# Starlight0798/gymRL

Measured on AMD Instinct MI355X. Metric: env-steps/sec at N envs/GPU (PPO LunarLander), 1/2/4/8 GPUs + %HBM roofline, higher is better.
Workload: dtype f32; 1 GPU; PPO LunarLander-v3, 4096 vectorised envs per MI355X (BASELINE.json configs[1]); envs_per_gpu=4096, rollout_len=2048, num_epochs=10, num_minibatches=32, minibatch=262144, model=ActorCritic 8-256-256-{256-4,256-1} tanh, 200,965 params, parallelism=single GPU

## Files before the change

### gymrl_amd/_lib.py

```python
import ctypes as C
import os
import subprocess

import torch

_HERE = os.path.dirname(os.path.abspath(__file__))
LIB_PATH = os.environ.get("GYMRL_HIP_LIB") or os.path.join(_HERE, "libgymrl_hip.so")
CSRC = os.path.join(_HERE, "csrc")

ABI_VERSION = 4

_lib = None

def build(force=False):
    if force:
        subprocess.check_call(["make", "-C", CSRC, "-s", "clean"])
    subprocess.check_call(["make", "-C", CSRC, "-s", "-j8"])
    return LIB_PATH


class LinItem(C.Structure):
    _c_name_ = "gymrl_lin_item"
    _fields_ = ([(n, C.c_void_p) for n in ("x", "x2", "w", "b", "y", "dy", "dx", "dx2", "dw", "db")] +
                [("act", C.c_int), ("lo", C.c_float), ("hi", C.c_float), ("argmax", C.c_void_p)])
# ... 533 lines not shown
    "gymrl_mhc_gates": (_i, [_vp, _vp, _vp, _vp, _vp, _i, _i, _i, _i, _vp, _vp, _vp, _vp, _vp, _vp]),
    "gymrl_mhc_combine": (_i, [_vp, _vp, _vp, _vp, _i, _i, _i, _i, _vp, _vp]),
    "gymrl_rmsnorm": (_i, [_vp, _vp, _i, _i, _i, _f, _i, _vp, _vp]),
    "gymrl_rmsnorm_bwd_workspace_bytes": (_sz, [_i]),
    "gymrl_rmsnorm_bwd": (_i, [_vp, _vp, _vp, _i, _i, _f, _i, _vp, _vp, _vp, _vp]),
    "gymrl_rmsnorm_sum_bwd": (_i, [_vp, _vp, _vp, _i, _i, _i, _f, _i, _vp, _vp, _vp, _vp]),
    "gymrl_norm_proj_fwd": (_i, [_vp, _vp, _vp, _vp, _i, _i, _i, _f, _vp, _vp]),
    "gymrl_norm_proj_bwd_workspace_bytes": (_sz, [_i, _i]),
    "gymrl_norm_proj_bwd": (_i, [_vp, _vp, _vp, _vp, _i, _i, _i, _f, _vp, _vp, _vp, _vp, _vp, _vp]),
    "gymrl_sinkhorn": (_i, [_vp, _i, _i, _i, _vp, _vp, _vp]),
    "gymrl_mhc_gates_bwd_workspace_bytes": (_sz, [_i, _i]),
    "gymrl_mhc_gates_bwd": (_i, [_vp, _vp, _vp, _vp, _vp, _vp, _vp, _vp, _vp, _vp, _vp, _vp, _vp, _i, _i, _i, _vp, _vp, _vp, _vp, _vp, _vp, _vp]),
    "gymrl_mhc_read_fwd": (_i, [_vp, _vp, _i, _i, _i, _vp, _vp]),
    "gymrl_mhc_read_bwd": (_i, [_vp, _vp, _vp, _i, _i, _i, _vp, _vp, _i, _vp]),
    "gymrl_mhc_combine_bwd": (_i, [_vp, _vp, _vp, _vp, _vp, _i, _i, _i, _i, _vp, _vp, _vp, _vp, _vp]),
    "gymrl_mhc_sub_forward": (_i, [_vp, _i, _vp, _vp, _vp, _vp, _vp, _vp, _i, _i, _i, _i, _vp, _vp, _vp, _vp, _vp, _vp, _vp, _vp]),
    "gymrl_mhc_sub_backward": (_i, [_vp, _i, _vp, _i, _vp, _vp, _vp, _vp, _vp, _vp, _vp, _vp, _vp, _i, _i, _i, _vp, _vp, _i, _vp, _vp, _vp, _vp, _vp,
                                    _vp]),
    "gymrl_mhc_policy_image_floats": (_sz, [_i]),
    "gymrl_mhc_policy_pack": (_i, [_vp, _vp, _vp]),
    "gymrl_mhc_policy_forward": (_i, [_vp, _vp, _i, _vp, _vp, _vp]),
    "gymrl_mlp_train_workspace_bytes": (_sz, [_i, _i, _i]),
    "gymrl_linear_tanh_smallk": (_i, [_vp, _vp, _vp, _i64, _i, _i, _vp, _vp]),
    "gymrl_linear_smallk": (_i, [_vp, _vp, _vp, _i64, _i, _i, _vp, _vp]),
    "gymrl_tanh_inplace": (_i, [_vp, _i64, _vp, _i, _vp]),
    "gymrl_tanh_bwd_colsum": (_i, [_vp, _vp, _i64, _i, _vp, _vp, _vp]),
    "gymrl_linear_smallk_bwd": (_i, [_vp, _vp, _vp, _i64, _i, _i, _vp, _vp, _vp, _vp, _vp, _vp]),
    "gymrl_heads_fwd_tanh": (_i, [_vp, _i64, _i, _i, _vp, _vp, _vp, _vp, _vp, _vp, _vp, _i, _vp]),
    "gymrl_heads_bwd": (_i, [_vp, _vp, _vp, _i64, _i, _i, _vp, _vp, _vp, _vp, _vp, _vp, _vp, _vp, _i, _vp, _vp, _vp]),
    "gymrl_heads_loss_blocks": (_i, [_i64, _i]),
    "gymrl_ppo_update_shape_ok": (_i, [_i, _i, _i]),
    "gymrl_heads_loss_fwd_bwd": (_i, [_vp, _i64, _i, _i, _vp, _vp, _vp, _vp, _vp, _vp, _vp, _vp, _vp, _vp, _P(PPOCfg), _vp, _vp, _vp, _vp, _vp, _vp,
                                      _vp, _vp]),
    "gymrl_ppo_gauss_update_shape_ok": (_i, [_i, _i, _i]),
    "gymrl_gauss_heads_loss_workspace_bytes": (_sz, [_i64, _i, _i]),
    "gymrl_gauss_heads_loss_fwd_bwd": (_i, [_vp, _i64, _i, _i, _vp, _vp, _vp, _vp, _vp, _vp, _vp, _vp, _vp, _vp, _vp, _P(PPOCfg), _vp, _vp, _vp,
                                            _vp, _vp, _vp, _vp, _vp, _vp, _i, _vp]),
    "gymrl_gemm_workspace_bytes": (_sz, []),
    "gymrl_linear_fwd": (_i, [_vp, _vp, _vp, _i64, _i, _i, _i, _vp, _vp]),
    "gymrl_linear_bwd_input": (_i, [_vp, _vp, _vp, _i64, _i, _i, _vp, _vp]),
    "gymrl_linear_bwd_input_add": (_i, [_vp, _vp, _vp, _i64, _i, _i, _vp, _vp]),
    "gymrl_linear_geometry": (_i, [_i, _i64, _i, _i, _P(_i), _P(_i)]),
    "gymrl_linear_bwd_weight_geometry": (_i, [_i64, _i, _P(_i), _P(_i64)]),
    "gymrl_linear_bwd_weight": (_i, [_vp, _vp, _i64, _i, _i, _vp, _vp, _vp, _vp]),
    "gymrl_update_finalize": (_i, [_i64, _i, _i, _i, _vp, _vp, _vp, _vp, _vp, _vp, _vp, _vp, _vp, _vp, _vp, _vp, _vp, _vp, _vp]),
    "gymrl_replay_append": (_i, [_vp, _vp, _vp, _vp, _vp, _i64, _i64, _i, _i, _i, _vp, _vp, _vp, _vp, _vp, _vp, _vp]),
# ... 130 lines not shown
```

### gymrl_amd/csrc/finalize_device.hpp

```cpp
#pragma once
#include "train_device.hpp"

namespace gymrl {
namespace fin {

constexpr int kCUs = 256;
constexpr size_t kColsumBytes = (size_t)kCUs * 512 * sizeof(float);

__host__ __device__ __forceinline__ void tn_geometry(int64_t B, int N, int* slices, int64_t* rps) {
  const int ntiles = N / 256;
  int s = kCUs / ntiles;
  int64_t r = (B + s - 1) / s;
  r += r & 1;
  if (r < 64) r = 64;
  s = (int)((B + r - 1) / r);
  if (s < 1) s = 1;
  *slices = s;
  *rps = r;
}

__device__ __forceinline__ void tn_colsum_body(const float* __restrict__ parts, int slices, float* __restrict__ db, int block,
                                               double (*sm)[64]) {
  const int n = block * 64 + (threadIdx.x & 63), j = threadIdx.x >> 6;
  const int ntile = n >> 8, nl = n & 255;
// ... 4 lines not shown
    float v[8];
#pragma unroll
    for (int k = 0; k < 8; ++k) v[k] = src[(size_t)(s + 4 * k) * 256];
#pragma unroll
    for (int k = 0; k < 8; ++k) g += (double)v[k];
  }
  for (; s < slices; s += 4) g += (double)src[(size_t)s * 256];
  sm[j][threadIdx.x & 63] = g;
  __syncthreads();
  if (j == 0) {
    const int l = threadIdx.x;
    db[n] = (float)(((sm[0][l] + sm[1][l]) + sm[2][l]) + sm[3][l]);
  }
}

__device__ __forceinline__ void tn_reduce_body(const float* __restrict__ parts, int slices, int ldw, float* __restrict__ dW,
                                               int block, double (*sm)[64][4]) {
  typedef float f32x4 __attribute__((ext_vector_type(4)));
  const int g = threadIdx.x >> 6, e = block * 64 + (threadIdx.x & 63);
  const int ntile = e >> 14, e4 = e & 16383;
  const f32x4* src = reinterpret_cast<const f32x4*>(parts) + (size_t)ntile * slices * 16384 + e4;
  double s0 = 0.0, s1 = 0.0, s2 = 0.0, s3 = 0.0;
  int s = g;
  for (; s + 12 < slices; s += 16) {
    const f32x4 v0 = src[(size_t)s * 16384], v1 = src[(size_t)(s + 4) * 16384];
    const f32x4 v2 = src[(size_t)(s + 8) * 16384], v3 = src[(size_t)(s + 12) * 16384];
    s0 += (double)v0[0]; s1 += (double)v0[1]; s2 += (double)v0[2]; s3 += (double)v0[3];
    s0 += (double)v1[0]; s1 += (double)v1[1]; s2 += (double)v1[2]; s3 += (double)v1[3];
    s0 += (double)v2[0]; s1 += (double)v2[1]; s2 += (double)v2[2]; s3 += (double)v2[3];
    s0 += (double)v3[0]; s1 += (double)v3[1]; s2 += (double)v3[2]; s3 += (double)v3[3];
  }
  for (; s < slices; s += 4) {
    const f32x4 v = src[(size_t)s * 16384];
    s0 += (double)v[0]; s1 += (double)v[1]; s2 += (double)v[2]; s3 += (double)v[3];
  }
  const int le = threadIdx.x & 63;
  if (g > 0) { sm[g - 1][le][0] = s0; sm[g - 1][le][1] = s1; sm[g - 1][le][2] = s2; sm[g - 1][le][3] = s3; }
  __syncthreads();
  if (g == 0) {
#pragma unroll
    for (int j = 0; j < 3; ++j) { s0 += sm[j][le][0]; s1 += sm[j][le][1]; s2 += sm[j][le][2]; s3 += sm[j][le][3]; }
    const int n = e4 >> 6, k4 = e4 & 63;
    *reinterpret_cast<f32x4*>(dW + (size_t)(ntile * 256 + n) * ldw + 4 * k4) = f32x4{(float)s0, (float)s1, (float)s2, (float)s3};
  }
}

}
}
```

### gymrl_amd/csrc/mlp_train.hip

```cpp
#include "train_device.hpp"
#include "finalize_device.hpp"
#include "policy_device.hpp"
#include "gauss_policy_device.hpp"
#include "../../include/gymrl.h"

namespace {

using namespace gymrl;

constexpr int kTB = 256;
constexpr int kMaxBlocks = 1024;

struct RowMap {
  int lpr, rpw, r_in, c4;
  __device__ RowMap(int C, int lane) : lpr(C >> 2), rpw(64 / (C >> 2)), r_in(lane / (C >> 2)), c4(lane % (C >> 2)) {}
};

inline int grid_for(int64_t rows, int C) {
  const int rows_per_block = (kTB / 64) * (64 / (C / 4));
  int64_t nb = (rows + rows_per_block - 1) / rows_per_block;
  return (int)(nb < kMaxBlocks ? (nb < 1 ? 1 : nb) : kMaxBlocks);
}

template <int NV>
__device__ __forceinline__ void block_colsum(const float (&acc)[NV], int C, const RowMap& m, float* sm,
                                             float* __restrict__ partials) {
  static_assert(NV % 4 == 0, "vectors of 4 columns");
  const int wave = threadIdx.x >> 6;
  const int groups = (kTB / 64) * m.rpw;
  const int g = wave * m.rpw + m.r_in;
  const int width = (NV / 4) * C;
#pragma unroll
  for (int v = 0; v < NV / 4; ++v)
#pragma unroll
    for (int j = 0; j < 4; ++j) sm[(size_t)g * width + v * C + 4 * m.c4 + j] = acc[4 * v + j];
  __syncthreads();
  for (int e = threadIdx.x; e < width; e += kTB) {
    float s = 0.0f;
    for (int gg = 0; gg < groups; ++gg) s += sm[(size_t)gg * width + e];
    partials[(size_t)blockIdx.x * width + e] = s;
  }
}

constexpr int kFinE = 32, kFinB = kTB / kFinE;
__device__ __forceinline__ double reduce_partials(const float* __restrict__ partials, int nblocks, int width, int e,
                                                  bool valid) {
  __shared__ double fin[kFinB][kFinE];
  const int te = threadIdx.x % kFinE, tb = threadIdx.x / kFinE;
  double s = 0.0;
  if (valid) {
    int b = tb;
    for (; b + 3 * kFinB < nblocks; b += 4 * kFinB) {
      const float p0 = partials[(size_t)b * width + e], p1 = partials[(size_t)(b + kFinB) * width + e];
      const float p2 = partials[(size_t)(b + 2 * kFinB) * width + e], p3 = partials[(size_t)(b + 3 * kFinB) * width + e];
      s += (double)p0; s += (double)p1; s += (double)p2; s += (double)p3;
    }
    for (; b < nblocks; b += kFinB) s += (double)partials[(size_t)b * width + e];
  }
  fin[tb][te] = s;
  __syncthreads();
  double t = 0.0;
  if (tb == 0) {
#pragma unroll
    for (int k = 0; k < kFinB; ++k) t += fin[k][te];
  }
  return t;
}

template <int D>
__device__ __forceinline__ void load_row(float (&xv)[D], const float* __restrict__ p) {
  if constexpr (D % 4 == 0) {
#pragma unroll
    for (int d = 0; d < D; d += 4) {
      const f32x4 v = *reinterpret_cast<const f32x4*>(p + d);
      xv[d] = v[0]; xv[d + 1] = v[1]; xv[d + 2] = v[2]; xv[d + 3] = v[3];
    }
  } else if constexpr (D == 6) {
#pragma unroll
// ... 12 lines not shown
                                                                 const float* __restrict__ b, int64_t B, int C,
                                                                 float* __restrict__ out) {
  const RowMap m(C, threadIdx.x & 63);
  float w[4][D], bias[4];
#pragma unroll
  for (int j = 0; j < 4; ++j) {
    bias[j] = b ? b[4 * m.c4 + j] : 0.0f;
#pragma unroll
    for (int d = 0; d < D; ++d) w[j][d] = W[(size_t)(4 * m.c4 + j) * D + d];
  }
  const int64_t stride = (int64_t)gridDim.x * (kTB / 64) * m.rpw;
  for (int64_t r = ((int64_t)blockIdx.x * (kTB / 64) + (threadIdx.x >> 6)) * m.rpw + m.r_in; r < B; r += stride) {
    float xv[D];
    load_row<D>(xv, x + r * D);
    f32x4 o;
#pragma unroll
    for (int j = 0; j < 4; ++j) {
      float acc = 0.0f;
#pragma unroll
      for (int d = 0; d < D; ++d) acc = fmaf(xv[d], w[j][d], acc);
      o[j] = TANH ? train_tanhf(acc + bias[j]) : acc + bias[j];
    }
    __builtin_nontemporal_store(o, reinterpret_cast<f32x4*>(out + r * C + 4 * m.c4));
  }
}

__global__ __launch_bounds__(kTB) void tanh_inplace_kernel(float* __restrict__ z, int64_t n4, const float* __restrict__ bias,
                                                           int C4) {
  f32x4* p = reinterpret_cast<f32x4*>(z);
  for (int64_t i = (int64_t)blockIdx.x * kTB + threadIdx.x; i < n4; i += (int64_t)gridDim.x * kTB) {
    f32x4 v = p[i];
    if (bias) {
      const f32x4 b = reinterpret_cast<const f32x4*>(bias)[i & (C4 - 1)];
#pragma unroll
      for (int j = 0; j < 4; ++j) v[j] += b[j];
    }
#pragma unroll
    for (int j = 0; j < 4; ++j) v[j] = train_tanhf(v[j]);
    p[i] = v;
  }
}

template <int A>
__global__ __launch_bounds__(kTB) void heads_fwd_tanh_kernel(float* __restrict__ Zac, int64_t B, int C,
                                                             const float* __restrict__ bac,
                                                             const float* __restrict__ Wa2, const float* __restrict__ ba2,
// ... 719 lines not shown

extern "C" {

size_t gymrl_mlp_train_workspace_bytes(int C, int D, int A) {
  if (C <= 0 || D < 0 || A < 0) return 0;
  const size_t w1 = (size_t)(D + 1) * C, w2 = (size_t)(3 + A + (A + 1 + 3) / 4) * C;
  return sizeof(float) * kMaxBlocks * (w1 > w2 ? w1 : w2) + 256;
}

int gymrl_linear_tanh_smallk(const float* x, const float* W, const float* b, int64_t B, int D, int C, float* out,
                             void* stream) {
  if (!x || !W || !out || B < 0 || !pow2_cols(C) || !al16(out) || !al16(x)) return -22;
  if (B == 0) return 0;
  const dim3 grid(grid_for(B, C) * 1), block(kTB);
  hipStream_t s = (hipStream_t)stream;
  switch (D) {
    case 2: hipLaunchKernelGGL(linear_tanh_smallk_kernel<2>, grid, block, 0, s, x, W, b, B, C, out); break;
    case 3: hipLaunchKernelGGL(linear_tanh_smallk_kernel<3>, grid, block, 0, s, x, W, b, B, C, out); break;
    case 4: hipLaunchKernelGGL(linear_tanh_smallk_kernel<4>, grid, block, 0, s, x, W, b, B, C, out); break;
    case 6: hipLaunchKernelGGL(linear_tanh_smallk_kernel<6>, grid, block, 0, s, x, W, b, B, C, out); break;
    case 8: hipLaunchKernelGGL(linear_tanh_smallk_kernel<8>, grid, block, 0, s, x, W, b, B, C, out); break;
    default: return -22;
  }
  GYMRL_CHECK_LAUNCH();
  return 0;
}

int gymrl_linear_smallk(const float* x, const float* W, const float* b, int64_t B, int D, int C, float* out, void* stream) {
  if (!x || !W || !out || B < 0 || !pow2_cols(C) || !al16(out) || !al16(x)) return -22;
  if (B == 0) return 0;
  const dim3 grid(grid_for(B, C) * 1), block(kTB);
  hipStream_t s = (hipStream_t)stream;
  switch (D) {
    case 2: hipLaunchKernelGGL((linear_tanh_smallk_kernel<2, false>), grid, block, 0, s, x, W, b, B, C, out); break;
    case 3: hipLaunchKernelGGL((linear_tanh_smallk_kernel<3, false>), grid, block, 0, s, x, W, b, B, C, out); break;
    case 4: hipLaunchKernelGGL((linear_tanh_smallk_kernel<4, false>), grid, block, 0, s, x, W, b, B, C, out); break;
    case 6: hipLaunchKernelGGL((linear_tanh_smallk_kernel<6, false>), grid, block, 0, s, x, W, b, B, C, out); break;
    case 8: hipLaunchKernelGGL((linear_tanh_smallk_kernel<8, false>), grid, block, 0, s, x, W, b, B, C, out); break;
    default: return -22;
  }
  GYMRL_CHECK_LAUNCH();
  return 0;
}

int gymrl_tanh_inplace(float* z, int64_t n, const float* bias, int C, void* stream) {
  if (!z || n < 0 || (n & 3) || !al16(z)) return -22;
// ... 182 lines not shown
```

### gymrl_amd/csrc/ppo.hip

```cpp
#include "gymrl_device.hpp"
#include "policy_device.hpp"
#include "gauss_policy_device.hpp"
#include "../../include/gymrl.h"

using namespace gymrl;

namespace {

constexpr int kBlock = 256;

template <int K, int BLOCK>
__device__ __forceinline__ void block_partials(double (&v)[K], double* __restrict__ partials) {
  __shared__ double sm[K][BLOCK / 64];
  const int lane = threadIdx.x & 63, wid = threadIdx.x >> 6;
#pragma unroll
  for (int k = 0; k < K; ++k) {
    const double s = wave_sum(v[k]);
    if (lane == 0) sm[k][wid] = s;
  }
  __syncthreads();
  if (threadIdx.x < K) {
    double s = 0.0;
#pragma unroll
    for (int w = 0; w < BLOCK / 64; ++w) s += sm[threadIdx.x][w];
    partials[(size_t)blockIdx.x * K + threadIdx.x] = s;
// ... 357 lines not shown
#pragma unroll
  for (int k = 0; k < K; ++k) v[k] = 0.0;
  for (int i = threadIdx.x; i < nblocks; i += kBlock) {
#pragma unroll
    for (int k = 0; k < K; ++k) v[k] += partials[(size_t)i * K + k];
  }
  const int lane = threadIdx.x & 63, wid = threadIdx.x >> 6;
#pragma unroll
  for (int k = 0; k < K; ++k) {
    const double s = wave_sum(v[k]);
    if (lane == 0) sm[k][wid] = s;
  }
  __syncthreads();
  if (threadIdx.x < K) {
    double s = 0.0;
#pragma unroll
    for (int w = 0; w < kBlock / 64; ++w) s += sm[threadIdx.x][w];
    metrics_sum[threadIdx.x] += s;
  }
}

constexpr int kMaxLossBlocks = 1024;

constexpr int kRecF = 16;

__global__ __launch_bounds__(kBlock) void permutation_kernel(uint64_t seed, uint64_t counter, uint32_t M, int a, int b,
                                                             int32_t* __restrict__ out) {
  const uint32_t i = blockIdx.x * kBlock + threadIdx.x;
  if (i < M) out[i] = (int32_t)keyed_permute(i, M, a, b, seed, counter);
}

__global__ __launch_bounds__(kBlock) void pack_rollout_kernel(
    const float* __restrict__ obs, const int32_t* __restrict__ act, const float* __restrict__ logp,
    const float* __restrict__ adv, const float* __restrict__ ret, int64_t M, int D,
    float* __restrict__ packed) {
  const int64_t stride = (int64_t)gridDim.x * kBlock;
  for (int64_t i = (int64_t)blockIdx.x * kBlock + threadIdx.x; i < M; i += stride) {
    float r[kRecF];
#pragma unroll
    for (int k = 0; k < 12; ++k) r[k] = k < D ? obs[i * D + k] : 0.0f;
    r[12] = __int_as_float(act[i]); r[13] = logp[i]; r[14] = adv[i]; r[15] = ret[i];
    float4* dst = reinterpret_cast<float4*>(packed + i * kRecF);
#pragma unroll
    for (int q = 0; q < 4; ++q) dst[q] = make_float4(r[4 * q], r[4 * q + 1], r[4 * q + 2], r[4 * q + 3]);
  }
}

__global__ __launch_bounds__(kBlock) void gather_minibatch_kernel(
    const float* __restrict__ packed, const int32_t* __restrict__ idx, int B, int D,
    float* __restrict__ obs_out, int32_t* __restrict__ act_out, float* __restrict__ logp_out,
    float* __restrict__ adv_out, float* __restrict__ ret_out) {
  for (int b = blockIdx.x * kBlock + threadIdx.x; b < B; b += gridDim.x * kBlock) {
    const float4* src = reinterpret_cast<const float4*>(packed + (size_t)idx[b] * kRecF);
    const float4 q0 = src[0], q1 = src[1], q2 = src[2], q3 = src[3];
    const float r[12] = {q0.x, q0.y, q0.z, q0.w, q1.x, q1.y, q1.z, q1.w, q2.x, q2.y, q2.z, q2.w};
    if (D == 8) {
      reinterpret_cast<float4*>(obs_out)[2 * (size_t)b] = q0;
      reinterpret_cast<float4*>(obs_out)[2 * (size_t)b + 1] = q1;
    } else if (D == 4) {
      reinterpret_cast<float4*>(obs_out)[b] = q0;
    } else {
#pragma unroll
      for (int k = 0; k < 12; ++k) if (k < D) obs_out[(size_t)b * D + k] = r[k];
    }
    act_out[b] = __float_as_int(q3.x); logp_out[b] = q3.y; adv_out[b] = q3.z; ret_out[b] = q3.w;
  }
}

__global__ __launch_bounds__(kBlock) void gather_rows_kernel(const float4* __restrict__ src, const int32_t* __restrict__ idx, int64_t n,
                                                             int quads, float4* __restrict__ out) {
  for (int64_t e = (int64_t)blockIdx.x * kBlock + threadIdx.x; e < n * quads; e += (int64_t)gridDim.x * kBlock) {
    const int64_t b = e / quads;
    const int q = (int)(e - b * quads);
    out[e] = src[(int64_t)idx[b] * quads + q];
  }
}

inline int cdiv(int a, int b) { return (a + b - 1) / b; }

}

#define DISPATCH_A(A_, CALL)              \
  switch (A_) {                           \
    case 2: { constexpr int A = 2; CALL; } break; \
    case 3: { constexpr int A = 3; CALL; } break; \
    case 4: { constexpr int A = 4; CALL; } break; \
    case 5: { constexpr int A = 5; CALL; } break; \
    case 6: { constexpr int A = 6; CALL; } break; \
    case 7: { constexpr int A = 7; CALL; } break; \
// ... 282 lines not shown
```

### gymrl_amd/ops.py

```python
import collections
import ctypes as C

import torch

from ._lib import (ACT_NONE, ACT_RELU, ACT_TANH, MLP_MAX_INPUT, MLP_MAX_STAGES, MLP_MAX_WIDTH, ClassicDuelEvalArgs, ClassicEvalArgs, ClassicPpoEvalArgs, DdqnUpdateArgs, EsNoiseArgs, EsPerturbArgs, EsShapeGradArgs, SnesPerturbArgs, SnesTellArgs, DqnActArgs, NdqnActArgs, NdqnCombineArgs, NdqnUpdateArgs, DqnUpdateArgs, DsacActArgs, DsacUpdateArgs, GaeOnline,
                   LunarCollectArgs, LunarEvalArgs, PendulumPpoEvalArgs, RolloutPendulumArgs, MlpDesc, MlpPackStackArgs, MlprnnParams, AcrobotNetEvalArgs, MountainCarEvalArgs, MountainCarNetEvalArgs, PPOCfg, PPOFullCfg, RainbowActArgs, RainbowUpdateArgs, RolloutLunarArgs, SacActArgs, SacUpdateArgs,
                   TabularTrainArgs, Td3ActArgs, Td3UpdateArgs, check, lib)

_vp = C.c_void_p


def _ptr(t, dtype=None, allow_none=False):
    if t is None:
        if allow_none:
            return _vp(None)
        raise ValueError("tensor required")
    if not t.is_cuda:
        raise RuntimeError("gymrl_amd ops run on the MI355X only: got a CPU tensor (there is no CPU fallback)")
    if dtype is not None and t.dtype != dtype:
        raise TypeError(f"expected {dtype}, got {t.dtype}")
    if not t.is_contiguous():
        raise ValueError("tensor must be contiguous")
    return _vp(t.data_ptr())

# ... 1502 lines not shown
        e.act, e.src, e.dst = int(st.get("act", ACT_NONE)), int(st["src"]), int(st["dst"])
        if e.dst < 0:
            if out is None or out.dim() != 2 or out.shape[1] != e.out_dim:
                raise ValueError("dst == -1 needs an `out` tensor [n_rows, out_dim]")
            e.out, e.out_stride = _ptr(out, torch.float32).value, out.stride(0)
    d._keepalive = list(stages)
    return d


def mlp_forward(x, desc):
    n, in_dim = x.shape
    check(lib().gymrl_mlp_forward(_ptr(x, torch.float32), n, in_dim, C.byref(desc), _stream()), "gymrl_mlp_forward")


def mlp_train_workspace(C_, D, A, device):
    n = lib().gymrl_mlp_train_workspace_bytes(C_, D, A)
    return torch.empty(n, dtype=torch.uint8, device=device)


def linear_tanh_smallk(x, W, b, out):
    B, D = x.shape
    check(lib().gymrl_linear_tanh_smallk(_ptr(x, torch.float32), _ptr(W, torch.float32), _ptr(b, torch.float32, True), B, D, W.shape[0],
                                         _ptr(out, torch.float32), _stream()), "gymrl_linear_tanh_smallk")
    return out


def linear_smallk(x, W, b, out):
    B, D = x.shape
    check(lib().gymrl_linear_smallk(_ptr(x, torch.float32), _ptr(W, torch.float32), _ptr(b, torch.float32, True), B, D, W.shape[0],
                                    _ptr(out, torch.float32), _stream()), "gymrl_linear_smallk")
    return out


def tanh_inplace(z, bias=None):
    check(lib().gymrl_tanh_inplace(_ptr(z, torch.float32), z.numel(), _ptr(bias, torch.float32, True), z.shape[-1], _stream()), "gymrl_tanh_inplace")
    return z


def tanh_bwd_colsum(dH, H, colsum_out, workspace):
    B, Cc = dH.shape
    check(lib().gymrl_tanh_bwd_colsum(_ptr(dH, torch.float32), _ptr(H, torch.float32), B, Cc, _ptr(colsum_out, torch.float32), _ptr(workspace),
                                      _stream()), "gymrl_tanh_bwd_colsum")
    return dH


def linear_smallk_bwd(dH, H, x, dW, db, workspace, W=None, b=None):
# ... 1275 lines not shown
```

### gymrl_amd/ppo_lunarlander.py

```python
from collections import deque

import numpy as np
import torch
import torch.nn as nn

from . import dist as gdist
from . import ops
from .envs import VecEnv
from .flat import FusedAdam, flatten_module
from . import ppo_net
from .nn import FusedMLP, Linear


class Config:
    def __init__(self):
        self.env_name = "LunarLander-v3"
        self.seed = None

        self.max_train_steps = 1_000_000
        self.update_freq = 2048
        self.num_epochs = 10
        self.batch_size = 64
        self.num_minibatches = None

# ... 182 lines not shown
        T = int(config.update_freq)
        self.buffer = self._build_buffer(T, N, state_dim)
        self.step_count = 0
        self.rollout_count = 0
        self.episode_rewards = deque(maxlen=100)
        self._gae_ws = ops.gae_workspace(T, N, self.device)
        self._moments = torch.zeros(3, dtype=torch.float64, device=self.device)
        self._next_value = torch.zeros(N, device=self.device)
        self._perm_seed, self._perm_draws, self._perm = self.base_seed * 7919 + 13 + self.rank, 0, None
        self._loss_cfg = (config.clip_eps, config.dual_clip, config.value_coef, config.entropy_coef)
        self._finished = None
        self._metric_parts = None
        self._agg_ready = self._carry_ready = False
        self._parity_noise = None
        self._parity_indices = []
        self._wg_ticks = None
        self._eval_env_factory = None
        self._gae_running = torch.zeros(2, N, dtype=torch.float64, device=self.device)
        self._packed = None
        mb = self._minibatch_size_for(T * N)
        self._stage = (torch.empty(mb, state_dim, device=self.device), torch.empty(mb, dtype=torch.int32, device=self.device),
                       torch.empty(mb, device=self.device), torch.empty(mb, device=self.device),
                       torch.empty(mb, device=self.device))
        self._stage2 = tuple(torch.empty_like(t) for t in self._stage) if self.collective else None
        self._reducer = None
        self._graph = None
        self._timers = None
        if self.rank == 0:
            print(f"Device: {self.device} x{self.world_size} | envs/GPU: {N} | rollout T: {T}")
            print(f"State dim: {state_dim}, Action dim: {action_dim}")
            print(f"Model parameters: {sum(p.numel() for p in self.model.parameters()):,}")

    def _action_dim(self):
        return self.env.action_space.n

    def _build_model(self, state_dim, action_dim):
        return ActorCritic(state_dim, action_dim, self.cfg.hidden_dim)

    def _build_buffer(self, T, N, state_dim):
        return RolloutBuffer(T, N, state_dim, self.device)

    def _sample_step(self, t, head, value, noise, counter0, online):
        b, env = self.buffer, self.env
        ops.categorical_sample(head, value=value.view(-1), noise_exp=None if noise is None else noise[t],
                               seed=env.seed, counter=counter0 + t,
                               env_id0=env.env_id0, act_out=b.actions[t], logp_out=b.log_probs[t],
                               ent_out=None, value_out=b.values[t], online=online)
# ... 175 lines not shown
                self._timers.stop("moments_allreduce", 3)
        total = len(b)
        mb = self._minibatch_size()
        n_mb = (total + mb - 1) // mb
        obs_dim = b.states.shape[-1]
        tm = self._timers
        self._packed = ops.pack_rollout(b.states[:b.T].reshape(total, obs_dim), self._packed_actions(),
                                        b.log_probs.view(-1), b.advantages.view(-1), b.returns.view(-1),
                                        self._packed)
        fu = self._fused_update_for(mb)
        one_pass = fu is not None
        nblk = fu.metric_blocks(mb) if one_pass else ops.loss_blocks(mb)
        if self._metric_parts is None or self._metric_parts.shape[:2] != (cfg.num_epochs * n_mb, nblk):
            self._metric_parts = torch.zeros(cfg.num_epochs * n_mb, nblk, 5, dtype=torch.float64, device=self.device)
        else:
            self._metric_parts.zero_()
        red = None
        if self.collective:
            if self._reducer is None:
                split = (self.model.actor[0].weight.data_ptr() - self.flat_params.data_ptr()) // 4
                self._reducer = gdist.GradReducer(self.flat_grads, [split] if one_pass else None)
            red = self._reducer
            red.timed = tm is not None
        stages = (self._stage, self._stage2) if red is not None else (self._stage, self._stage)

        def minibatches():
            for epoch in range(cfg.num_epochs):
                if indices is not None:
                    perm = torch.as_tensor(indices[epoch], device=self.device).to(torch.int32)
                else:
                    self._perm_draws += 1
                    self._perm = ops.permutation(self._perm_seed, self._perm_draws, total, self.device,
                                                 out=self._perm if self._perm is not None and self._perm.numel() == total else None)
                    perm = self._perm
                for start in range(0, total, mb):
                    yield perm[start:start + mb]

        def gather(mb_idx, k):
            B = mb_idx.numel()
            if tm is not None:
                tm.start("gather_minibatch")
            out = ops.gather_minibatch(self._packed, mb_idx, obs_dim, stages[k & 1] if B == mb else None)
            if tm is not None:
                tm.stop("gather_minibatch", B)
            return out

        graphed = (one_pass and red is None and bool(getattr(cfg, "use_graphs", False)) and total % mb == 0
                   and cfg.num_epochs * n_mb > 3)
        gs = self._graph_state(fu, mb, obs_dim) if graphed else None

        sizes = []
        row = 0
        it = minibatches()
        first = next(it)
        cur = gather(first, 0) if not graphed else first
        while cur is not None:
            if tm is not None:
                tm.tick()
            if graphed:
                mb_idx = cur
                B = mb_idx.numel()
                if tm is not None and tm.live:
                    fu.timers = tm
                    g5 = gather(mb_idx, 0)
                    fu.step(*g5, self._loss_cfg, self._moments, self._metric_parts[row])
                    tm.start("adam_step")
                    self.optimizer.step(grad_scale=1.0)
                    tm.stop("adam_step", self.flat_params.numel())
                else:
                    fu.timers = None
                    gs["idx"].copy_(mb_idx)
                    gs["scalars"].set(gs["off"], self.optimizer.next_bias())
                    gs["scalars"].flush()
                    gs["step"]()
                    self._metric_parts[row].copy_(gs["metric"])
                sizes.append(B)
                row += 1
                cur = next(it, None)
                continue
            mb_obs, mb_act, mb_lp, mb_adv, mb_ret = cur
            B = mb_obs.shape[0]
            if one_pass:
                fu.step(mb_obs, mb_act, mb_lp, mb_adv, mb_ret, self._loss_cfg, self._moments, self._metric_parts[row],
                        reducer=red)
            else:
                self._loss_backward(mb_obs, mb_act, mb_lp, mb_adv, mb_ret, row, tm)
                if red is not None:
                    red.launch(0)
            nxt = next(it, None)
            cur = gather(nxt, row + 1) if nxt is not None else None
            if red is not None:
                red.wait()
            if tm is not None:
                tm.start("adam_step")
            self.optimizer.step(grad_scale=1.0 / self.world_size)
            if tm is not None:
                tm.stop("adam_step", self.flat_params.numel())
            sizes.append(B)
            row += 1
        if tm is not None:
            tm.resume()
        metrics = ops.reduce_rows(self._metric_parts, row, nblk, 5)
        self._drain_episode_returns()
        m = metrics.cpu().numpy() / np.asarray(sizes, np.float64)[:, None]
        m = m.mean(axis=0)
        return {"policy_loss": m[0], "value_loss": m[1], "entropy": m[2], "clip_frac": m[3], "approx_kl": m[4]}

    def _graph_state(self, fu, mb, obs_dim):
        key = (id(fu), mb, self._packed.data_ptr(), self._stage[0].data_ptr())
        gs = self._graph
        if gs is None or gs["key"] != key:
            from .graphs import GraphedStep, StepScalars
            sc = StepScalars(self.device)
            bias, off = sc.slot(16, torch.float32)
            gs = self._graph = dict(key=key, scalars=sc, bias=bias, off=off,
                                    idx=torch.empty(mb, dtype=torch.int32, device=self.device),
                                    metric=torch.zeros(fu.metric_blocks(mb), 5, dtype=torch.float64, device=self.device))

            def body():
                g5 = ops.gather_minibatch(self._packed, gs["idx"], obs_dim, self._stage)
                fu.step(*g5, self._loss_cfg, self._moments, gs["metric"])
                self.optimizer.step(grad_scale=1.0, bias_dev=gs["bias"])
            gs["step"] = GraphedStep(body, warmup=2)
        return gs

    def save_checkpoint(self, path):
        from .utils import checkpoint
        return checkpoint.save_agent(path, {"model": self.model}, {"optimizer": (self.model, self.optimizer)},
                                     step_count=self.step_count, rollout_count=self.rollout_count,
                                     perm_draws=self._perm_draws, episode_rewards=list(self.episode_rewards))

    def load_checkpoint(self, path):
        from .utils import checkpoint
        rest = checkpoint.load_agent(path, {"model": self.model}, {"optimizer": (self.model, self.optimizer)})
        self.step_count = int(rest.get("step_count", 0))
        self.rollout_count = int(rest.get("rollout_count", 0))
        self._perm_draws = int(rest.get("perm_draws", 0))
        self.episode_rewards.clear()
        self.episode_rewards.extend(rest.get("episode_rewards", []))
        gdist.broadcast(self.flat_params)
        return rest

    def train(self):
        if self.rank == 0:
# ... 116 lines not shown
```

### gymrl_amd/ppo_net.py

```python
import torch

from . import ops

LAYOUT = ["shared.0.weight", "shared.0.bias", "shared.2.weight", "shared.2.bias",
          "actor.0.weight", "critic.0.weight", "actor.0.bias", "critic.0.bias",
          "actor.2.weight", "actor.2.bias", "critic.2.weight", "critic.2.bias"]


def supported(model):
    H = model.shared[0].out_features
    D = model.shared[0].in_features
    A = model.actor[2].out_features
    return (ops.ppo_update_shape_ok(H, D, A)
            and model.shared[2].out_features == H and model.actor[0].out_features == H
            and model.critic[0].out_features == H)


def gauss_supported(model):
    H = model.shared[0].out_features
    D = model.shared[0].in_features
    A = model.actor[2].out_features
    return (ops.ppo_gauss_update_shape_ok(H, D, A)
            and model.shared[2].out_features == H and model.actor[0].out_features == H
            and model.critic[0].out_features == H and hasattr(model, "log_std"))
# ... 15 lines not shown
        if wc.data_ptr() != wa.data_ptr() + wa.numel() * 4 or bc.data_ptr() != ba.data_ptr() + ba.numel() * 4:
            raise ValueError("actor.0 / critic.0 are not adjacent: flatten_module(model, device, order=ppo_net.LAYOUT)")
        flat, gflat = model._flat_params, model._flat_grads

        def view(p, n, shape, buf):
            off = (p.data_ptr() - flat.data_ptr()) // 4
            return buf[off:off + n].view(shape)
        self.Wac = view(wa, 2 * H * H, (2 * H, H), flat)
        self.bac = view(ba, 2 * H, (2 * H,), flat)
        self.dWac = view(wa, 2 * H * H, (2 * H, H), gflat)
        self.dbac = view(ba, 2 * H, (2 * H,), gflat)
        self.ws = ops.mlp_train_workspace(H, self.D, self.A, dev)
        R = int(max_rows)
        self.R = R
        self.H1 = torch.empty(R, H, device=dev)
        self.H2 = torch.empty(R, H, device=dev)
        self.Hac = torch.empty(R, 2 * H, device=dev)
        self.dH2 = torch.empty(R, H, device=dev)
        self.dH1 = torch.empty(R, H, device=dev)
        self.timers = None
        self.one_pass_heads, defer = self._schedule()
        self.gemm_ws = ops.gemm_workspace(dev) if H == 256 else None
        self.defer_finalize = defer
        self.gemm_ws2 = ops.gemm_workspace(dev) if defer else None
        self.ws2 = ops.mlp_train_workspace(H, self.D, self.A, dev) if defer else None
        if not self.one_pass_heads:
            self.logits = torch.empty(R, self.A, device=dev)
            self.value = torch.empty(R, 1, device=dev)
            self.dlogits = torch.empty(R, self.A, device=dev)
            self.dvalue = torch.empty(R, device=dev)
        if H != 256:
            self.lin_ws = ops.lin_workspace(R, 2 * H, H, 1, dev) if R > 512 else None

    def _schedule(self):
        return self.H == 256 or self.A == 3, self.H == 256

    def _heads_one_pass(self, t, sfx, B, Zac, heads, act, logp_old, adv, ret, loss_cfg, adv_moments, dbac, hg, metric_parts):
        t("heads_loss_fwd_bwd" + sfx, B, ops.heads_loss_fwd_bwd, Zac, None, *heads, act, logp_old, adv, ret, loss_cfg, adv_moments,
          dbac, *hg, metric_parts, self.ws)

    def _timed(self, name, units, fn, *args, **kw):
        tm = self.timers
        if tm is None:
            return fn(*args, **kw)
        tm.start(name)
        r = fn(*args, **kw)
        tm.stop(name, units)
        return r

    def metric_blocks(self, B):
        return ops.heads_loss_blocks(B, self.H) if self.one_pass_heads else ops.loss_blocks(B)

    @torch.no_grad()
    def step(self, x, act, logp_old, adv, ret, loss_cfg, adv_moments, metric_parts, reducer=None):
        m, B, H = self.m, x.shape[0], self.H
        if B > self.R:
            raise ValueError("minibatch larger than the buffers")
        t = self._timed
        H1, H2, Zac, dZ2, dZ1 = self.H1[:B], self.H2[:B], self.Hac[:B], self.dH2[:B], self.dH1[:B]
        W2, ws = m.shared[2].weight, self.gemm_ws
        sfx = "" if H == 256 else f"_h{H}"
        t("linear_tanh_smallk", B, ops.linear_tanh_smallk, x, m.shared[0].weight, m.shared[0].bias, H1)
        t(f"gemm_fwd_{H}_tanh", B, ops.linear_fwd, H1, W2, m.shared[2].bias, H2, True)
        t(f"gemm_fwd_{2 * H}", B, ops.linear_fwd, H2, self.Wac, self.bac, Zac, False)
        heads = (m.actor[2].weight, m.actor[2].bias, m.critic[2].weight, m.critic[2].bias)
        hgrads = (m.actor[2].weight.grad, m.actor[2].bias.grad, m.critic[2].weight.grad, m.critic[2].bias.grad)
        wide = H == 256
        defer = self.defer_finalize and self.one_pass_heads and wide and reducer is None
        if self.one_pass_heads:
            dbac, hg = (None, (None,) * 4) if defer else (self.dbac, hgrads)
            self._heads_one_pass(t, sfx, B, Zac, heads, act, logp_old, adv, ret, loss_cfg, adv_moments, dbac, hg, metric_parts)
        else:
            logits, value, dl, dv = self.logits[:B], self.value[:B], self.dlogits[:B], self.dvalue[:B]
            t("heads_fwd_tanh" + sfx, B, ops.heads_fwd_tanh, Zac, heads[0], heads[1], heads[2], heads[3], logits, value, None, False)
            t("ppo_loss_fwd_bwd" + sfx, B, ops.ppo_loss_fwd_bwd, logits, value.view(-1), act, logp_old, adv, ret, loss_cfg,
              adv_moments=adv_moments, dlogits_out=dl, dvalue_out=dv, workspace=metric_parts)
            t("heads_bwd" + sfx, B, ops.heads_bwd, Zac, dl, dv, heads[0], heads[2], Zac, self.dbac, hgrads[0], hgrads[1],
              hgrads[2], hgrads[3], self.ws, True, None)
        if wide:
            t("gemm_dw_512", B, ops.linear_bwd_weight, Zac, H2, None if defer else self.dWac, ws)
        else:
            t(f"lin_dw_{2 * H}", B, ops.lin_bwd_weight, Zac, None, H2, self.dWac, workspace=self.lin_ws)
        if reducer is not None:
            reducer.launch(1)
        t(f"gemm_dx_{2 * H}_tanhbwd", B, ops.linear_bwd_input, Zac, self.Wac, H2, dZ2)
# ... 38 lines not shown
```

### include/gymrl.h

```cpp
#ifndef GYMRL_H
#define GYMRL_H

#include <stddef.h>
#include <stdint.h>

#ifdef __cplusplus
extern "C" {
#endif

#define GYMRL_ABI_VERSION 4

int gymrl_abi_version(void);
int gymrl_device_ok(void);

enum {
  GYMRL_ENV_CARTPOLE    = 0,
  GYMRL_ENV_PENDULUM    = 1,
  GYMRL_ENV_LUNARLANDER = 2,
  GYMRL_ENV_MOUNTAINCAR = 3,
  GYMRL_ENV_ACROBOT     = 5
};
#define GYMRL_ACROBOT_WRAP_TRIPS 8


// ... 445 lines not shown
  const float* b1;
  const float* norm_w;
  float norm_eps;
  const float* w2;
  const float* b2;
} gymrl_mhc_head;
typedef struct gymrl_mhc_policy_s {
  int obs_dim, n_sub, n_act, sk_it;
  const float* in_w;
  const float* in_b;
  gymrl_mhc_sub sub[8];
  const float* final_norm_w;
  float final_norm_eps;
  gymrl_mhc_head head[2];
  const float* image;
} gymrl_mhc_policy;
size_t gymrl_mhc_policy_image_floats(int n_sub);
int gymrl_mhc_policy_pack(const gymrl_mhc_policy* p, float* image, void* stream);
int gymrl_mhc_policy_forward(const gymrl_mhc_policy* p, const float* obs, int B, float* logits_out, float* value_out, void* stream);

size_t gymrl_mlp_train_workspace_bytes(int C, int D, int A);
int gymrl_linear_tanh_smallk(const float* x, const float* W, const float* b, int64_t B, int D, int C,
                             float* out, void* stream);
int gymrl_linear_smallk(const float* x, const float* W, const float* b, int64_t B, int D, int C, float* out, void* stream);
int gymrl_tanh_inplace(float* z, int64_t n, const float* bias, int C, void* stream);
int gymrl_tanh_bwd_colsum(float* dH, const float* H, int64_t B, int C, float* colsum_out,
                          void* workspace, void* stream);
int gymrl_linear_smallk_bwd(const float* dH, const float* H, const float* x, int64_t B, int D, int C,
                            float* dW, float* db, const float* W, const float* b, void* workspace,
                            void* stream);
int gymrl_heads_fwd_tanh(float* Zac, int64_t B, int C, int A, const float* bac, const float* Wa2,
                         const float* ba2, const float* Wc2, const float* bc2, float* logits, float* value,
                         int store_h, void* stream);
int gymrl_heads_bwd(const float* Hac, const float* dlogits, const float* dv, int64_t B, int C, int A,
                    const float* Wa2, const float* Wc2, float* dZac, float* dbac, float* dWa2,
                    float* dba2, float* dWc2, float* dbc2, int pre_activation, const float* bac,
                    void* workspace, void* stream);

int gymrl_heads_loss_blocks(int64_t B, int C);
int gymrl_ppo_update_shape_ok(int C, int D, int A);
int gymrl_heads_loss_fwd_bwd(float* Zac, int64_t B, int C, int A, const float* bac, const float* Wa2,
                             const float* ba2, const float* Wc2, const float* bc2, const int32_t* act,
                             const float* logp_old, const float* adv, const float* ret,
                             const double* adv_moments, const gymrl_ppo_cfg* cfg, float* dbac, float* dWa2,
                             float* dba2, float* dWc2, float* dbc2, double* metric_parts, void* workspace,
                             void* stream);
// ... 564 lines not shown
```

Baseline: 7.333 million env-steps/s.

## Fuse minibatch gather into first-layer linear-tanh kernel via index lookup

```diff
diff --git a/gymrl_amd/_lib.py b/gymrl_amd/_lib.py
--- a/gymrl_amd/_lib.py
+++ b/gymrl_amd/_lib.py
@@ -579,6 +579,7 @@
     "gymrl_mhc_policy_forward": (_i, [_vp, _vp, _i, _vp, _vp, _vp]),
     "gymrl_mlp_train_workspace_bytes": (_sz, [_i, _i, _i]),
     "gymrl_linear_tanh_smallk": (_i, [_vp, _vp, _vp, _i64, _i, _i, _vp, _vp]),
+    "gymrl_linear_tanh_smallk_indexed": (_i, [_vp, _vp, _vp, _vp, _i64, _i, _i, _vp, _vp, _vp, _vp, _vp, _vp, _vp]),
     "gymrl_linear_smallk": (_i, [_vp, _vp, _vp, _i64, _i, _i, _vp, _vp]),
     "gymrl_tanh_inplace": (_i, [_vp, _i64, _vp, _i, _vp]),
     "gymrl_tanh_bwd_colsum": (_i, [_vp, _vp, _i64, _i, _vp, _vp, _vp]),
diff --git a/gymrl_amd/csrc/finalize_device.hpp b/gymrl_amd/csrc/finalize_device.hpp
--- a/gymrl_amd/csrc/finalize_device.hpp
+++ b/gymrl_amd/csrc/finalize_device.hpp
@@ -50,13 +50,12 @@
   const f32x4* src = reinterpret_cast<const f32x4*>(parts) + (size_t)ntile * slices * 16384 + e4;
   double s0 = 0.0, s1 = 0.0, s2 = 0.0, s3 = 0.0;
   int s = g;
-  for (; s + 12 < slices; s += 16) {
-    const f32x4 v0 = src[(size_t)s * 16384], v1 = src[(size_t)(s + 4) * 16384];
-    const f32x4 v2 = src[(size_t)(s + 8) * 16384], v3 = src[(size_t)(s + 12) * 16384];
-    s0 += (double)v0[0]; s1 += (double)v0[1]; s2 += (double)v0[2]; s3 += (double)v0[3];
-    s0 += (double)v1[0]; s1 += (double)v1[1]; s2 += (double)v1[2]; s3 += (double)v1[3];
-    s0 += (double)v2[0]; s1 += (double)v2[1]; s2 += (double)v2[2]; s3 += (double)v2[3];
-    s0 += (double)v3[0]; s1 += (double)v3[1]; s2 += (double)v3[2]; s3 += (double)v3[3];
+  for (; s + 28 < slices; s += 32) {
+    f32x4 v[8];
+#pragma unroll
+    for (int k = 0; k < 8; ++k) v[k] = src[(size_t)(s + 4 * k) * 16384];
+#pragma unroll
+    for (int k = 0; k < 8; ++k) { s0 += (double)v[k][0]; s1 += (double)v[k][1]; s2 += (double)v[k][2]; s3 += (double)v[k][3]; }
   }
   for (; s < slices; s += 4) {
     const f32x4 v = src[(size_t)s * 16384];
diff --git a/gymrl_amd/csrc/minibatch_device.hpp b/gymrl_amd/csrc/minibatch_device.hpp
--- /dev/null
+++ b/gymrl_amd/csrc/minibatch_device.hpp
@@ -0,0 +1,41 @@
+#pragma once
+#include "gymrl_device.hpp"
+
+namespace gymrl {
+namespace mbrec {
+
+constexpr int kRecF = 16;
+
+struct Record { float4 q0, q1, q2, q3; };
+
+__device__ __forceinline__ Record load_record(const float* __restrict__ packed, int32_t row) {
+  const float4* src = reinterpret_cast<const float4*>(packed + (size_t)row * kRecF);
+  return Record{src[0], src[1], src[2], src[3]};
+}
+
+__device__ __forceinline__ void store_staged(const Record& q, size_t b, int D, float* __restrict__ obs_out,
+                                             int32_t* __restrict__ act_out, float* __restrict__ logp_out,
+                                             float* __restrict__ adv_out, float* __restrict__ ret_out) {
+  if (D == 8) {
+    reinterpret_cast<float4*>(obs_out)[2 * b] = q.q0;
+    reinterpret_cast<float4*>(obs_out)[2 * b + 1] = q.q1;
+  } else if (D == 4) {
+    reinterpret_cast<float4*>(obs_out)[b] = q.q0;
+  } else {
+    const float r[12] = {q.q0.x, q.q0.y, q.q0.z, q.q0.w, q.q1.x, q.q1.y, q.q1.z, q.q1.w, q.q2.x, q.q2.y, q.q2.z, q.q2.w};
+#pragma unroll
+    for (int k = 0; k < 12; ++k) if (k < D) obs_out[b * D + k] = r[k];
+  }
+  act_out[b] = __float_as_int(q.q3.x); logp_out[b] = q.q3.y; adv_out[b] = q.q3.z; ret_out[b] = q.q3.w;
+}
+
+template <int D>
+__device__ __forceinline__ void record_obs(float (&x)[D], const Record& q) {
+  static_assert(D <= 8, "first layers with at most 8 inputs");
+  const float r[8] = {q.q0.x, q.q0.y, q.q0.z, q.q0.w, q.q1.x, q.q1.y, q.q1.z, q.q1.w};
+#pragma unroll
+  for (int d = 0; d < D; ++d) x[d] = r[d];
+}
+
+}
+}
diff --git a/gymrl_amd/csrc/mlp_train.hip b/gymrl_amd/csrc/mlp_train.hip
--- a/gymrl_amd/csrc/mlp_train.hip
+++ b/gymrl_amd/csrc/mlp_train.hip
@@ -1,5 +1,6 @@
 #include "train_device.hpp"
 #include "finalize_device.hpp"
+#include "minibatch_device.hpp"
 #include "policy_device.hpp"
 #include "gauss_policy_device.hpp"
 #include "../../include/gymrl.h"
@@ -42,7 +43,7 @@
   }
 }
 
-constexpr int kFinE = 32, kFinB = kTB / kFinE;
+constexpr int kFinE = 32, kFinB = kTB / kFinE, kFinU = 16;
 __device__ __forceinline__ double reduce_partials(const float* __restrict__ partials, int nblocks, int width, int e,
                                                   bool valid) {
   __shared__ double fin[kFinB][kFinE];
@@ -50,10 +51,12 @@
   double s = 0.0;
   if (valid) {
     int b = tb;
-    for (; b + 3 * kFinB < nblocks; b += 4 * kFinB) {
-      const float p0 = partials[(size_t)b * width + e], p1 = partials[(size_t)(b + kFinB) * width + e];
-      const float p2 = partials[(size_t)(b + 2 * kFinB) * width + e], p3 = partials[(size_t)(b + 3 * kFinB) * width + e];
-      s += (double)p0; s += (double)p1; s += (double)p2; s += (double)p3;
+    for (; b + (kFinU - 1) * kFinB < nblocks; b += kFinU * kFinB) {
+      float p[kFinU];
+#pragma unroll
+      for (int k = 0; k < kFinU; ++k) p[k] = partials[(size_t)(b + k * kFinB) * width + e];
+#pragma unroll
+      for (int k = 0; k < kFinU; ++k) s += (double)p[k];
     }
     for (; b < nblocks; b += kFinB) s += (double)partials[(size_t)b * width + e];
   }
@@ -112,6 +115,50 @@
       o[j] = TANH ? train_tanhf(acc + bias[j]) : acc + bias[j];
     }
     __builtin_nontemporal_store(o, reinterpret_cast<f32x4*>(out + r * C + 4 * m.c4));
+  }
+}
+
+template <int D>
+__global__ __launch_bounds__(kTB) void linear_tanh_smallk_indexed_kernel(
+    const float* __restrict__ packed, const int32_t* __restrict__ idx, const float* __restrict__ W, const float* __restrict__ b,
+    int64_t B, float* __restrict__ out, float* __restrict__ obs_out, int32_t* __restrict__ act_out,
+    float* __restrict__ logp_out, float* __restrict__ adv_out, float* __restrict__ ret_out) {
+  constexpr int C = 256;
+  const int lane = threadIdx.x & 63;
+  const int wave = __builtin_amdgcn_readfirstlane(threadIdx.x >> 6);
+  float w[4][D], bias[4];
+#pragma unroll
+  for (int j = 0; j < 4; ++j) {
+    bias[j] = b ? b[4 * lane + j] : 0.0f;
+#pragma unroll
+    for (int d = 0; d < D; ++d) w[j][d] = W[(size_t)(4 * lane + j) * D + d];
+  }
+  const int64_t nchunks = (B + 63) / 64;
+  for (int64_t ch = (int64_t)blockIdx.x * (kTB / 64) + wave; ch < nchunks; ch += (int64_t)gridDim.x * (kTB / 64)) {
+    const int64_t r0 = ch * 64;
+    float xl[D];
+#pragma unroll
+    for (int d = 0; d < D; ++d) xl[d] = 0.0f;
+    if (r0 + lane < B) {
+      const mbrec::Record q = mbrec::load_record(packed, idx[r0 + lane]);
+      mbrec::store_staged(q, (size_t)(r0 + lane), D, obs_out, act_out, logp_out, adv_out, ret_out);
+      mbrec::record_obs<D>(xl, q);
+    }
+    const int n = (int)(B - r0 < 64 ? B - r0 : 64);
+    for (int i = 0; i < n; ++i) {
+      float xv[D];
+#pragma unroll
+      for (int d = 0; d < D; ++d) xv[d] = __int_as_float(__builtin_amdgcn_readlane(__float_as_int(xl[d]), i));
+      f32x4 o;
+#pragma unroll
+      for (int j = 0; j < 4; ++j) {
+        float acc = 0.0f;
+#pragma unroll
+        for (int d = 0; d < D; ++d) acc = fmaf(xv[d], w[j][d], acc);
+        o[j] = train_tanhf(acc + bias[j]);
+      }
+      __builtin_nontemporal_store(o, reinterpret_cast<f32x4*>(out + (r0 + i) * C + 4 * lane));
+    }
   }
 }
 
@@ -877,6 +924,30 @@
     case 8: hipLaunchKernelGGL(linear_tanh_smallk_kernel<8>, grid, block, 0, s, x, W, b, B, C, out); break;
     default: return -22;
   }
+  GYMRL_CHECK_LAUNCH();
+  return 0;
+}
+
+int gymrl_linear_tanh_smallk_indexed(const float* packed, const int32_t* idx, const float* W, const float* b, int64_t B, int D,
+                                     int C, float* out, float* obs_out, int32_t* act_out, float* logp_out, float* adv_out,
+                                     float* ret_out, void* stream) {
+  if (!packed || !idx || !W || !out || !obs_out || !act_out || !logp_out || !adv_out || !ret_out || B < 0 || B > INT32_MAX ||
+      C != 256 || !update_obs(D) || !al16(packed) || !al16(out) || !al16(obs_out))
+    return -22;
+  if (B == 0) return 0;
+  const int64_t want = ((B + 63) / 64 + (kTB / 64) - 1) / (kTB / 64);
+  const dim3 grid((unsigned)(want < 2 * kMaxBlocks ? want : 2 * kMaxBlocks)), block(kTB);
+  hipStream_t s = (hipStream_t)stream;
+#define GYMRL_IDX_ARGS grid, block, 0, s, packed, idx, W, b, B, out, obs_out, act_out, logp_out, adv_out, ret_out
+  switch (D) {
+    case 2: hipLaunchKernelGGL(linear_tanh_smallk_indexed_kernel<2>, GYMRL_IDX_ARGS); break;
+    case 3: hipLaunchKernelGGL(linear_tanh_smallk_indexed_kernel<3>, GYMRL_IDX_ARGS); break;
+    case 4: hipLaunchKernelGGL(linear_tanh_smallk_indexed_kernel<4>, GYMRL_IDX_ARGS); break;
+    case 6: hipLaunchKernelGGL(linear_tanh_smallk_indexed_kernel<6>, GYMRL_IDX_ARGS); break;
+    case 8: hipLaunchKernelGGL(linear_tanh_smallk_indexed_kernel<8>, GYMRL_IDX_ARGS); break;
+    default: return -22;
+  }
+#undef GYMRL_IDX_ARGS
   GYMRL_CHECK_LAUNCH();
   return 0;
 }
diff --git a/gymrl_amd/csrc/ppo.hip b/gymrl_amd/csrc/ppo.hip
--- a/gymrl_amd/csrc/ppo.hip
+++ b/gymrl_amd/csrc/ppo.hip
@@ -1,6 +1,7 @@
 #include "gymrl_device.hpp"
 #include "policy_device.hpp"
 #include "gauss_policy_device.hpp"
+#include "minibatch_device.hpp"
 #include "../../include/gymrl.h"
 
 using namespace gymrl;
@@ -404,7 +405,7 @@
 
 constexpr int kMaxLossBlocks = 1024;
 
-constexpr int kRecF = 16;
+using mbrec::kRecF;
 
 __global__ __launch_bounds__(kBlock) void permutation_kernel(uint64_t seed, uint64_t counter, uint32_t M, int a, int b,
                                                              int32_t* __restrict__ out) {
@@ -432,21 +433,8 @@
     const float* __restrict__ packed, const int32_t* __restrict__ idx, int B, int D,
     float* __restrict__ obs_out, int32_t* __restrict__ act_out, float* __restrict__ logp_out,
     float* __restrict__ adv_out, float* __restrict__ ret_out) {
-  for (int b = blockIdx.x * kBlock + threadIdx.x; b < B; b += gridDim.x * kBlock) {
-    const float4* src = reinterpret_cast<const float4*>(packed + (size_t)idx[b] * kRecF);
-    const float4 q0 = src[0], q1 = src[1], q2 = src[2], q3 = src[3];
-    const float r[12] = {q0.x, q0.y, q0.z, q0.w, q1.x, q1.y, q1.z, q1.w, q2.x, q2.y, q2.z, q2.w};
-    if (D == 8) {
-      reinterpret_cast<float4*>(obs_out)[2 * (size_t)b] = q0;
-      reinterpret_cast<float4*>(obs_out)[2 * (size_t)b + 1] = q1;
-    } else if (D == 4) {
-      reinterpret_cast<float4*>(obs_out)[b] = q0;
-    } else {
-#pragma unroll
-      for (int k = 0; k < 12; ++k) if (k < D) obs_out[(size_t)b * D + k] = r[k];
-    }
-    act_out[b] = __float_as_int(q3.x); logp_out[b] = q3.y; adv_out[b] = q3.z; ret_out[b] = q3.w;
-  }
+  for (int b = blockIdx.x * kBlock + threadIdx.x; b < B; b += gridDim.x * kBlock)
+    mbrec::store_staged(mbrec::load_record(packed, idx[b]), (size_t)b, D, obs_out, act_out, logp_out, adv_out, ret_out);
 }
 
 __global__ __launch_bounds__(kBlock) void gather_rows_kernel(const float4* __restrict__ src, const int32_t* __restrict__ idx, int64_t n,
diff --git a/gymrl_amd/ops.py b/gymrl_amd/ops.py
--- a/gymrl_amd/ops.py
+++ b/gymrl_amd/ops.py
@@ -1548,6 +1548,17 @@
     B, D = x.shape
     check(lib().gymrl_linear_tanh_smallk(_ptr(x, torch.float32), _ptr(W, torch.float32), _ptr(b, torch.float32, True), B, D, W.shape[0],
                                          _ptr(out, torch.float32), _stream()), "gymrl_linear_tanh_smallk")
+    return out
+
+
+def linear_tanh_smallk_indexed(packed, idx, W, b, out, stage):
+    B = idx.numel()
+    obs, act, logp, adv, ret = stage
+    check(lib().gymrl_linear_tanh_smallk_indexed(_ptr(packed, torch.float32), _ptr(idx, torch.int32), _ptr(W, torch.float32),
+                                                 _ptr(b, torch.float32, True), B, W.shape[1], W.shape[0], _ptr(out, torch.float32),
+                                                 _ptr(obs, torch.float32), _ptr(act, torch.int32), _ptr(logp, torch.float32),
+                                                 _ptr(adv, torch.float32), _ptr(ret, torch.float32), _stream()),
+          "gymrl_linear_tanh_smallk_indexed")
     return out
 
 
diff --git a/gymrl_amd/ppo_lunarlander.py b/gymrl_amd/ppo_lunarlander.py
--- a/gymrl_amd/ppo_lunarlander.py
+++ b/gymrl_amd/ppo_lunarlander.py
@@ -228,7 +228,7 @@
         self._stage = (torch.empty(mb, state_dim, device=self.device), torch.empty(mb, dtype=torch.int32, device=self.device),
                        torch.empty(mb, device=self.device), torch.empty(mb, device=self.device),
                        torch.empty(mb, device=self.device))
-        self._stage2 = tuple(torch.empty_like(t) for t in self._stage) if self.collective else None
+        self._stage2 = None
         self._reducer = None
         self._graph = None
         self._timers = None
@@ -450,6 +450,9 @@
                 self._reducer = gdist.GradReducer(self.flat_grads, [split] if one_pass else None)
             red = self._reducer
             red.timed = tm is not None
+        indexed = one_pass and fu.takes_indices
+        if red is not None and not indexed and self._stage2 is None:
+            self._stage2 = tuple(torch.empty_like(t) for t in self._stage)
         stages = (self._stage, self._stage2) if red is not None else (self._stage, self._stage)
 
         def minibatches():
@@ -473,6 +476,13 @@
                 tm.stop("gather_minibatch", B)
             return out
 
+        def fused_step(mb_idx, metric, **kw):
+            if indexed:
+                stage = (t[:mb_idx.numel()] for t in self._stage)
+                fu.step(*stage, self._loss_cfg, self._moments, metric, packed=self._packed, idx=mb_idx, **kw)
+            else:
+                fu.step(*gather(mb_idx, 0), self._loss_cfg, self._moments, metric, **kw)
+
         graphed = (one_pass and red is None and bool(getattr(cfg, "use_graphs", False)) and total % mb == 0
                    and cfg.num_epochs * n_mb > 3)
         gs = self._graph_state(fu, mb, obs_dim) if graphed else None
@@ -481,7 +491,7 @@
         row = 0
         it = minibatches()
         first = next(it)
-        cur = gather(first, 0) if not graphed else first
+        cur = first if graphed or indexed else gather(first, 0)
         while cur is not None:
             if tm is not None:
                 tm.tick()
@@ -490,8 +500,7 @@
                 B = mb_idx.numel()
                 if tm is not None and tm.live:
                     fu.timers = tm
-                    g5 = gather(mb_idx, 0)
-                    fu.step(*g5, self._loss_cfg, self._moments, self._metric_parts[row])
+                    fused_step(mb_idx, self._metric_parts[row])
                     tm.start("adam_step")
                     self.optimizer.step(grad_scale=1.0)
                     tm.stop("adam_step", self.flat_params.numel())
@@ -506,17 +515,21 @@
                 row += 1
                 cur = next(it, None)
                 continue
-            mb_obs, mb_act, mb_lp, mb_adv, mb_ret = cur
-            B = mb_obs.shape[0]
-            if one_pass:
-                fu.step(mb_obs, mb_act, mb_lp, mb_adv, mb_ret, self._loss_cfg, self._moments, self._metric_parts[row],
-                        reducer=red)
+            if indexed:
+                B = cur.numel()
+                fused_step(cur, self._metric_parts[row], reducer=red)
             else:
-                self._loss_backward(mb_obs, mb_act, mb_lp, mb_adv, mb_ret, row, tm)
-                if red is not None:
-                    red.launch(0)
+                mb_obs, mb_act, mb_lp, mb_adv, mb_ret = cur
+                B = mb_obs.shape[0]
+                if one_pass:
+                    fu.step(mb_obs, mb_act, mb_lp, mb_adv, mb_ret, self._loss_cfg, self._moments, self._metric_parts[row],
+                            reducer=red)
+                else:
+                    self._loss_backward(mb_obs, mb_act, mb_lp, mb_adv, mb_ret, row, tm)
+                    if red is not None:
+                        red.launch(0)
             nxt = next(it, None)
-            cur = gather(nxt, row + 1) if nxt is not None else None
+            cur = None if nxt is None else nxt if indexed else gather(nxt, row + 1)
             if red is not None:
                 red.wait()
             if tm is not None:
@@ -546,8 +559,11 @@
                                     metric=torch.zeros(fu.metric_blocks(mb), 5, dtype=torch.float64, device=self.device))
 
             def body():
-                g5 = ops.gather_minibatch(self._packed, gs["idx"], obs_dim, self._stage)
-                fu.step(*g5, self._loss_cfg, self._moments, gs["metric"])
+                if fu.takes_indices:
+                    fu.step(*self._stage, self._loss_cfg, self._moments, gs["metric"], packed=self._packed, idx=gs["idx"])
+                else:
+                    g5 = ops.gather_minibatch(self._packed, gs["idx"], obs_dim, self._stage)
+                    fu.step(*g5, self._loss_cfg, self._moments, gs["metric"])
                 self.optimizer.step(grad_scale=1.0, bias_dev=gs["bias"])
             gs["step"] = GraphedStep(body, warmup=2)
         return gs
diff --git a/gymrl_amd/ppo_net.py b/gymrl_amd/ppo_net.py
--- a/gymrl_amd/ppo_net.py
+++ b/gymrl_amd/ppo_net.py
@@ -61,6 +61,7 @@
         self.one_pass_heads, defer = self._schedule()
         self.gemm_ws = ops.gemm_workspace(dev) if H == 256 else None
         self.defer_finalize = defer
+        self.takes_indices = defer
         self.gemm_ws2 = ops.gemm_workspace(dev) if defer else None
         self.ws2 = ops.mlp_train_workspace(H, self.D, self.A, dev) if defer else None
         if not self.one_pass_heads:
@@ -91,15 +92,25 @@
         return ops.heads_loss_blocks(B, self.H) if self.one_pass_heads else ops.loss_blocks(B)
 
     @torch.no_grad()
-    def step(self, x, act, logp_old, adv, ret, loss_cfg, adv_moments, metric_parts, reducer=None):
-        m, B, H = self.m, x.shape[0], self.H
+    def step(self, x, act, logp_old, adv, ret, loss_cfg, adv_moments, metric_parts, reducer=None, packed=None, idx=None):
+        m, H = self.m, self.H
+        if idx is not None:
+            if not self.takes_indices:
+                raise ValueError("this schedule takes gathered minibatches (ops.gather_minibatch)")
+            B = idx.numel()
+            x, act, logp_old, adv, ret = (s[:B] for s in (x, act, logp_old, adv, ret))
+        B = x.shape[0]
         if B > self.R:
             raise ValueError("minibatch larger than the buffers")
         t = self._timed
         H1, H2, Zac, dZ2, dZ1 = self.H1[:B], self.H2[:B], self.Hac[:B], self.dH2[:B], self.dH1[:B]
         W2, ws = m.shared[2].weight, self.gemm_ws
         sfx = "" if H == 256 else f"_h{H}"
-        t("linear_tanh_smallk", B, ops.linear_tanh_smallk, x, m.shared[0].weight, m.shared[0].bias, H1)
+        if idx is not None:
+            t("linear_tanh_smallk", B, ops.linear_tanh_smallk_indexed, packed, idx, m.shared[0].weight, m.shared[0].bias, H1,
+              (x, act, logp_old, adv, ret))
+        else:
+            t("linear_tanh_smallk", B, ops.linear_tanh_smallk, x, m.shared[0].weight, m.shared[0].bias, H1)
         t(f"gemm_fwd_{H}_tanh", B, ops.linear_fwd, H1, W2, m.shared[2].bias, H2, True)
         t(f"gemm_fwd_{2 * H}", B, ops.linear_fwd, H2, self.Wac, self.bac, Zac, False)
         heads = (m.actor[2].weight, m.actor[2].bias, m.critic[2].weight, m.critic[2].bias)
diff --git a/include/gymrl.h b/include/gymrl.h
--- a/include/gymrl.h
+++ b/include/gymrl.h
@@ -491,6 +491,9 @@
 size_t gymrl_mlp_train_workspace_bytes(int C, int D, int A);
 int gymrl_linear_tanh_smallk(const float* x, const float* W, const float* b, int64_t B, int D, int C,
                              float* out, void* stream);
+int gymrl_linear_tanh_smallk_indexed(const float* packed, const int32_t* idx, const float* W, const float* b, int64_t B, int D,
+                                     int C, float* out, float* obs_out, int32_t* act_out, float* logp_out, float* adv_out,
+                                     float* ret_out, void* stream);
 int gymrl_linear_smallk(const float* x, const float* W, const float* b, int64_t B, int D, int C, float* out, void* stream);
 int gymrl_tanh_inplace(float* z, int64_t n, const float* bias, int C, void* stream);
 int gymrl_tanh_bwd_colsum(float* dH, const float* H, int64_t B, int C, float* colsum_out,
```

After: 7.334 million env-steps/s, median of 2. About the same (+0.0%).
